# wenyuqing/panacea

Measured on AMD Instinct MI355X. Metric: denoising steps/s (6-view x 8-frame 256x512), higher is better.
Workload: dtype f16; 1 GPU; BASELINE config 3: Panacea+ stage-2 UNet+ControlNet, CFG 2 x 8 frames, 6 views, latent 32x384, hint 256x3072, Euler/LegacyDDPM 50-step schedule; precision=precise: split(stream,gn_stt,ff_out,stem,gn_head,gnt)+e4m3-lo, parallelism=single, graph=False, streams=2, hoisted_step_invariants=False, fused_step_tail=True

## Files before the change

### panacea_amd/build.py

```python
from __future__ import annotations

import hashlib
import os
import shutil
import subprocess
import sys
from pathlib import Path

PKG = Path(__file__).resolve().parent
ROOT = PKG.parent
CSRC = PKG / "csrc"
LIBDIR = PKG / "lib"
LIB = LIBDIR / "libpanacea_hip.so"
SOURCES = ["gemm.hip", "gemm_plain.hip", "gemm_conv3x3.hip", "gemm_stencil_tile.hip", "gemm_conv1d.hip", "attn.hip", "attn_split.hip", "norm.hip", "misc.hip"]
HEADERS = [CSRC / "common.h", CSRC / "gemm_kernel.h", ROOT / "include" / "panacea_hip.h"]
FLAGS = ["--offload-arch=gfx950", "-O3", "-std=c++17", "-fPIC", "-Wall", "-Wno-unused-function",
         "-I", str(ROOT / "include"), "-I", str(CSRC)]


def _hipcc() -> str:
    for cand in (os.environ.get("HIPCC"), shutil.which("hipcc"), "/opt/rocm/bin/hipcc"):
        if cand and Path(cand).exists():
            return cand
    raise RuntimeError("hipcc not found (expected /opt/rocm/bin/hipcc)")


def _digest() -> str:
    h = hashlib.sha256()
    for f in [CSRC / s for s in SOURCES] + HEADERS:
        h.update(f.read_bytes())
    h.update(" ".join(f.replace(str(ROOT), "<root>") for f in FLAGS).encode())
    return h.hexdigest()


def library_digest(lib: Path = LIB):
    try:
        blob = Path(lib).read_bytes()
    except OSError:
        return None
    i = blob.find(_DIGEST_MARK)
    if i < 0:
        return None
    j = blob.find(b"\0", i)
    return blob[i + len(_DIGEST_MARK):j].decode(errors="replace")


_DIGEST_MARK = b"pnc-build-digest:"
# ... 40 lines not shown
```

### panacea_amd/csrc/gemm.hip

```cpp
#include "gemm_kernel.h"
#include <math.h>
#include <mutex>

namespace pnc_gemm {

int dispatch_plain(const PncGemmParams& p, unsigned epi, hipStream_t st, bool* ln_fused);
int dispatch_conv3x3(const PncGemmParams& p, unsigned epi, hipStream_t st);
int dispatch_conv1d(const PncGemmParams& p, unsigned epi, hipStream_t st);

__device__ __attribute__((aligned(16))) float g_phi_table[2 * PHI_N];

const float* phi_table_device(hipStream_t st, int* rc) {
    static std::mutex mu;
    static const float* dev_ptr[64] = {};
    int dev = 0;
    (void)hipGetDevice(&dev);
    std::lock_guard<std::mutex> lock(mu);
    const float*& ptr = dev_ptr[dev & 63];
    *rc = PNC_OK;
    if (ptr) return ptr;
    hipStreamCaptureStatus cs = hipStreamCaptureStatusNone;
    if (hipStreamIsCapturing(st, &cs) == hipSuccess && cs != hipStreamCaptureStatusNone) { *rc = PNC_EINVAL; return nullptr; }
    static float host[2 * PHI_N];
    auto phi = [](double x) { return 0.5 * (1.0 + erf(x * 0.70710678118654752440)); };
    for (int i = 0; i < PHI_N; ++i) {
        const double x0 = (double)PHI_X0 + (double)i / PHI_SCALE, x1 = (double)PHI_X0 + (double)(i + 1) / PHI_SCALE;
        host[2 * i] = (float)phi(x0);
        host[2 * i + 1] = (float)(phi(x1) - phi(x0));
    }
    void* d = nullptr;
    if (hipMemcpyToSymbol(HIP_SYMBOL(g_phi_table), host, sizeof(host)) != hipSuccess ||
        hipGetSymbolAddress(&d, HIP_SYMBOL(g_phi_table)) != hipSuccess) {
        *rc = (int)hipGetLastError();
        return nullptr;
    }
    ptr = reinterpret_cast<const float*>(d);
    return ptr;
}

__global__ __launch_bounds__(256) void splitk_reduce_kernel(const PncGemmParams p, const int ksplit) {
    const int n8 = p.N >> 3;
// ... 126 lines not shown
    if (p.a_mode != PNC_A_CONV3X3 && p.x_halo_off) return PNC_EINVAL;
    if (p.gn_part && (p.a_mode != PNC_A_CONV1D_T || !p.out32 || (p.N % 64) || (p.ldc32 % 4) || p.out16t || p.geglu)) return PNC_EINVAL;
    if (p.act != PNC_ACT_NONE && p.act != PNC_ACT_SILU && p.act != PNC_ACT_GELU) return PNC_EINVAL;
    if (p.ldw != 0 && (p.ldw < p.K || p.ldw % 8)) return PNC_EALIGN;
    if (p.rowbias && (p.rb_rows <= 0 || p.rb_mod <= 0)) return PNC_EINVAL;
    if (p.geglu) {
        if ((p.N % 64) || p.out16t || p.out32 || p.res1 || p.res2 || p.rowbias || p.act != PNC_ACT_NONE || !p.out16)
            return PNC_EINVAL;
        if ((p.ldc16 % 8) || !al16(p.out16) || (p.out16_lo && !al16(p.out16_lo)) || (p.bias && !al16(p.bias)))
            return PNC_EALIGN;
    }
    if (p.out16t && ((p.n_split % 128) || p.t_rows <= 0 || p.N <= 32)) return PNC_EINVAL;
    if (p.out16_lo && !p.out16) return PNC_EINVAL;
    if ((p.a_lo_fmt != PNC_LO_F16 && p.a_lo_fmt != PNC_LO_E4M3) || (p.out_lo_fmt != PNC_LO_F16 && p.out_lo_fmt != PNC_LO_E4M3))
        return PNC_EINVAL;
    if (p.out16_lo && p.out_lo_fmt == PNC_LO_E4M3 && p.geglu) return PNC_EINVAL;
    if (p.A_lo && p.a_lo_fmt == PNC_LO_E4M3) {
        if (!p.W_lo || p.w_lo_exp < 1 || p.w_lo_exp > 254) return PNC_EINVAL;
        if ((uintptr_t)p.W_lo & 15) return PNC_EALIGN;
        if (p.K % 16 || (p.ldw_lo != 0 && (p.ldw_lo < p.K || p.ldw_lo % 16))) return PNC_EALIGN;
        if (p.a_mode == PNC_A_PLAIN ? (p.lda % 16 != 0) : (p.Cin % 64 != 0)) return PNC_EALIGN;
    }
    if (!p.out32 && !p.out16 && !p.out16t) return PNC_EINVAL;
    if (p.ln_out16) {
        if (!p.out32 || p.geglu || p.out16t || !p.ln_gamma || !p.ln_beta) return PNC_EINVAL;
        if (p.N % 4 || p.N > 4 * 64 * 12 || p.ldc32 % 4 || p.ldln % 4 || p.ldln < p.N) return PNC_EINVAL;
        if (!al16(p.out32) || !al16(p.ln_gamma) || !al16(p.ln_beta) || (((uintptr_t)p.ln_out16) & 7)) return PNC_EALIGN;
    }
    return PNC_OK;
}

extern "C" int pnc_abi_version(void) { return PNC_ABI_VERSION; }

extern "C" int64_t pnc_gemm_workspace_floats(const PncGemmParams* pp) {
    if (!pp || pp->struct_bytes != (int32_t)sizeof(PncGemmParams)) return 0;
    if (pp->M <= 0 || pp->N <= 0 || pp->K <= 0) return 0;
    if (pp->N <= 32 && !pp->geglu) return 0;
    const int ks = splitk_slices(*pp);
    return ks > 1 ? (int64_t)ks * pp->M * pp->N : 0;
}

static unsigned epilogue_with_ln(const PncGemmParams& p) {
    unsigned epi = select_epilogue(p);
    if (p.ln_out16 && p.a_mode == PNC_A_PLAIN && (epi == E_O32 || epi == (E_RB | E_O32) || epi == (E_R1 | E_O32)) &&
        (p.ldln % 8 == 0) && al16(p.ln_out16) && (pnc_get_option(PNC_OPT_GEMM_FUSE_LN) & 1))
        epi |= E_LN;
    return epi;
}

static void normalise(PncGemmParams& p) {
    if (!p.out16t) p.n_split = p.N;
    if (p.ldw == 0) p.ldw = p.K;
    if (p.ldw_lo == 0) p.ldw_lo = p.K;
    if (!p.res1 && p.res2) { p.res1 = p.res2; p.ldr1 = p.ldr2; p.res2 = nullptr; }
}

extern "C" int pnc_gemm_fuses_layernorm(const PncGemmParams* pp) {
    if (!pp || validate(*pp) != PNC_OK || !pp->ln_out16) return 0;
    PncGemmParams p = *pp;
    normalise(p);
    if (!(epilogue_with_ln(p) & E_LN)) return 0;
    const TileChoice tc = choose_tile(p);
    return ln_whole_rows(p, tc) ? 1 : 0;
}

extern "C" int pnc_gemm_f16(const PncGemmParams* pp, void* stream) {
    if (!pp) return PNC_EINVAL;
    const int rc = validate(*pp);
    if (rc != PNC_OK) return rc;
    PncGemmParams p = *pp;
    normalise(p);
    const unsigned epi = epilogue_with_ln(p);
// ... 15 lines not shown
```

### panacea_amd/csrc/gemm_conv1d.hip

```cpp
#include "gemm_kernel.h"

namespace pnc_gemm {

static bool gn_stats_in_epilogue(const PncGemmParams& p, const TileChoice& tc) {
    const int cpg = p.N / 32;
    return tc.tile == T_256x320 && (p.N % 320) == 0 && (160 % cpg) == 0 && (cpg % 2) == 0 && (p.Npix % 64) == 0 && (p.M % 64) == 0 &&
           pnc_get_option(PNC_OPT_GEMM_GN_STATS) != 0;
}

int dispatch_conv1d(const PncGemmParams& p, unsigned epi, hipStream_t st) {
    constexpr int AM = PNC_A_CONV1D_T;
    TileChoice tc = choose_tile(p);
    if (tc.tile == T_128x32) epi = E_GENERIC;
    if (p.gn_part) {
        int rc = PNC_EINVAL;
        bool fused = gn_stats_in_epilogue(p, tc);
        if (fused) {
            switch (epi) {
                case E_R1 | E_RB | E_O32: rc = launch<AM, 256, 320, 4, 2, 2, false, E_R1 | E_RB | E_O32 | E_GS>(p, st); break;
                case E_R1 | E_R2 | E_O32: rc = launch<AM, 256, 320, 4, 2, 2, false, E_R1 | E_R2 | E_O32 | E_GS>(p, st); break;
                case E_R1 | E_R2 | E_O32 | E_O16: rc = launch<AM, 256, 320, 4, 2, 2, false, E_R1 | E_R2 | E_O32 | E_O16 | E_GS>(p, st); break;
                default: fused = false;
            }
        }
        if (fused) return rc;
        PncGemmParams q = p;
        q.gn_part = nullptr;
        rc = dispatch_conv1d(q, epi, st);
        if (rc != PNC_OK) return rc;
        return pnc_groupnorm_stats(p.out32, p.ldc32, p.M / p.Npix, p.Npix, p.N, 64, p.gn_part, st);
    }
    switch (epi) {
        case E_R1 | E_RB | E_O32: return launch_tile<AM, E_R1 | E_RB | E_O32>(p, st, tc);
        case E_R1 | E_R2 | E_O32: return launch_tile<AM, E_R1 | E_R2 | E_O32>(p, st, tc);
        case E_R1 | E_R2 | E_O32 | E_O16: return launch_tile<AM, E_R1 | E_R2 | E_O32 | E_O16>(p, st, tc);
        default: return launch_tile<AM, E_GENERIC>(p, st, tc);
    }
}

}

PNC_DEFINE_TU_COLLECT(gemm_conv1d)
```

### panacea_amd/csrc/gemm_kernel.h

```cpp
#pragma once
#include "common.h"
#include <atomic>
#include <utility>

namespace pnc_gemm {

constexpr int BK = 64;
constexpr int BK8 = 128;
typedef int i32x4 __attribute__((ext_vector_type(4)));
typedef int i32x8 __attribute__((ext_vector_type(8)));
constexpr int E8M0_LO_INV = 127 - 11;

enum : unsigned {
    E_R1 = 1,
    E_R2 = 2,
    E_RB = 4,
    E_O32 = 8,
    E_O16 = 16,
    E_VT = 32,
    E_GEGLU = 64,
    E_GENERIC = 128,
    E_GELU = 256,
    E_LN = 512,
    E_GS = 1024
// ... 114 lines not shown
    for (int e = 0; e < 8; ++e) o[e] = (half_t)v[e];
    *reinterpret_cast<half8v*>(out16 + off) = o;
    if (out16_lo) {
        float r[8];
#pragma unroll
        for (int e = 0; e < 8; ++e) r[e] = (v[e] - (float)o[e]) * LO_SCALE;
        if (lo_fmt == PNC_LO_E4M3) {
            uint2 w;
            w.x = pack4_e4m3(r[0], r[1], r[2], r[3]);
            w.y = pack4_e4m3(r[4], r[5], r[6], r[7]);
            *reinterpret_cast<uint2*>(reinterpret_cast<char*>(out16_lo) + off) = w;
        } else {
            half8v l;
#pragma unroll
            for (int e = 0; e < 8; ++e) l[e] = (half_t)r[e];
            *reinterpret_cast<half8v*>(reinterpret_cast<half_t*>(out16_lo) + off) = l;
        }
    }
}

struct RowLinear {
    int mw;
    __device__ __forceinline__ int operator()(int lr) const { return mw + lr; }
};
template <int TWS>
struct RowHalo {
    int base, W, lr0;
    __device__ __forceinline__ int operator()(int lr) const {
        const int R = lr0 + lr;
        return base + (R >> TWS) * W + (R & ((1 << TWS) - 1));
    }
};

template <int MI, int NI, unsigned EPI, class RM = RowLinear>
__device__ __forceinline__ void epi_fast(const PncGemmParams& p, f32x16 (&acc)[MI][NI], float* ep, int lane,
                                         RM rmap, int nw, int ncols, float2* ln_mine = nullptr,
                                         const float2* ln_partner = nullptr, float* gs_tab = nullptr) {
    constexpr bool R1 = (EPI & E_R1) != 0, R2 = (EPI & E_R2) != 0, RB = (EPI & E_RB) != 0;
    constexpr bool O32 = (EPI & E_O32) != 0, O16 = (EPI & E_O16) != 0, LN = (EPI & E_LN) != 0;
    constexpr bool GS = (EPI & E_GS) != 0;
    static_assert(!GS || (O32 && !LN), "statistics of the fp32 output; not next to the fused LayerNorm");
    const int cpg = GS ? (p.N >> 5) : 1;
    if constexpr (GS) {
        gs_tab[lane] = 0.0f;
        if (lane + 64 < NI * 16) gs_tab[lane + 64] = 0.0f;
    }
    static_assert(!LN || O32, "the fused LayerNorm normalises the fp32 output it has just written");
    constexpr bool HAS_X = R1 || RB, HAS_Y = R1 && (R2 || RB);
    static_assert(!(R2 && !R1), "a single residual is passed as res1");
    static_assert(!(R1 && R2 && RB), "three added streams run the generic epilogue");
    constexpr int ENI = NI < 2 ? NI : 2;
    constexpr int EPITCH = ENI * 32 + 4;
    constexpr int NJ = (NI + ENI - 1) / ENI, NS = NJ * MI;
    constexpr int NPMAX = ENI == 2 ? 4 : 2;
    half_t* out16 = reinterpret_cast<half_t*>(p.out16);
    void* out16_lo = p.out16_lo;
    constexpr bool GELU = (EPI & E_GELU) != 0;
    const bool silu = (!HAS_X) && (p.act == PNC_ACT_SILU);
    const f32x4 z4 = {0.0f, 0.0f, 0.0f, 0.0f};
    f32x4 x0[NPMAX], x1[NPMAX], y0[NPMAX], y1[NPMAX];
    if constexpr (LN) {
        if (lane < MI * 32) ln_mine[lane] = make_float2(0.0f, 0.0f);
    }

    auto load_xy = [&](auto s_, auto ps_) {
        constexpr int s = decltype(s_)::value, ps = decltype(ps_)::value;
        constexpr int jc = (s / MI) * ENI, i = s % MI, cw = (NI - jc) < ENI ? (NI - jc) : ENI;
        constexpr int CPL = cw * 4, RPP = 64 / CPL;
        const int cl = lane % CPL, rl = lane / CPL;
        const int ncol = nw + jc * 32 + cl * 8;
        const int m = rmap(i * 32 + ps * RPP + rl);
        const bool on = (m < p.M) && (ncol < ncols);
        if constexpr (HAS_X) {
            x0[ps] = z4; x1[ps] = z4;
            if (on) {
                const float* xp = R1 ? p.res1 + (int64_t)m * p.ldr1 + ncol
                                     : p.rowbias + (int64_t)((m / p.rb_rows) % p.rb_mod) * p.N + ncol;
                x0[ps] = ld4(xp); x1[ps] = ld4(xp + 4);
// ... 85 lines not shown
            if constexpr (GS) {
                if (on) {
#pragma unroll
                    for (int k = 0; k < 4; ++k) {
                        gP[k] += v[2 * k] + v[2 * k + 1];
                        gQ[k] += fmaf(v[2 * k], v[2 * k], v[2 * k + 1] * v[2 * k + 1]);
                    }
                }
            }
            if (!on) return;
            if constexpr (O32) {
                float* op = p.out32 + (int64_t)m * p.ldc32 + ncol;
                const f32x4 o0 = {v[0], v[1], v[2], v[3]}, o1 = {v[4], v[5], v[6], v[7]};
                *reinterpret_cast<f32x4*>(op) = o0;
                *reinterpret_cast<f32x4*>(op + 4) = o1;
            }
            if constexpr (O16) store_h8(out16, out16_lo, (int64_t)m * p.ldc16 + ncol, v, p.out_lo_fmt);
        });
        if constexpr (GS) {
            const int nA = min(8, (ncol / cpg + 1) * cpg - ncol);
            float sA = 0.0f, qA = 0.0f, sB = 0.0f, qB = 0.0f;
#pragma unroll
            for (int k = 0; k < 4; ++k) {
                const bool a = 2 * k < nA;
                sA += a ? gP[k] : 0.0f; qA += a ? gQ[k] : 0.0f;
                sB += a ? 0.0f : gP[k]; qB += a ? 0.0f : gQ[k];
            }
#pragma unroll
            for (int o = CPL; o < 64; o <<= 1) {
                sA += __shfl_xor(sA, o, 64); qA += __shfl_xor(qA, o, 64);
                sB += __shfl_xor(sB, o, 64); qB += __shfl_xor(qB, o, 64);
            }
            if (lane < CPL) {
                f32x4* e = reinterpret_cast<f32x4*>(gs_tab + (jc * 4 + cl) * 4);
                f32x4 t = *e;
                t[0] += sA; t[1] += qA; t[2] += sB; t[3] += qB;
                *e = t;
            }
        }
        if constexpr (LN) {
            asm volatile("s_waitcnt lgkmcnt(0)" ::: "memory");
            static_for<cw>([&](auto j_) {
                constexpr int j = decltype(j_)::value;
#pragma unroll
                for (int r = 0; r < 16; ++r)
                    acc[i][jc + j][r] = ep[mfma32_row(r, lane) * EPITCH + j * 32 + (lane & 31)];
            });
        }
    });
    if constexpr (GS) {
        asm volatile("s_waitcnt lgkmcnt(0)" ::: "memory");
        const int m_first = rmap(0);
        if (lane < (NI * 32) / cpg && m_first < p.M) {
            const int c0 = (lane * cpg) >> 3, c1 = ((lane + 1) * cpg - 1) >> 3;
            float S = 0.0f, Q = 0.0f;
            for (int c = c0; c <= c1; ++c) {
                const f32x4 t = *reinterpret_cast<const f32x4*>(gs_tab + c * 4);
                const bool first = (c * 8) / cpg == lane;
                S += first ? t[0] : t[2];
                Q += first ? t[1] : t[3];
            }
            const float n = (float)(MI * 32 * cpg);
            const float mean = S / n;
            const int f = m_first / p.Npix, chunk = (m_first - f * p.Npix) / (MI * 32), nrec = p.Npix / (MI * 32);
            float* o = p.gn_part + ((int64_t)(f * nrec + chunk) * 32 + nw / cpg + lane) * 3;
            o[0] = n; o[1] = mean; o[2] = fmaxf(Q - S * mean, 0.0f);
        }
    }
    if constexpr (LN) {
        __syncthreads();
        half_t* lnout = reinterpret_cast<half_t*>(p.ln_out16);
        const float invn = 1.0f / (float)p.N;
        static_for<NS>([&](auto s_) {
            constexpr int s = decltype(s_)::value, jc = (s / MI) * ENI, i = s % MI;
            constexpr int cw = (NI - jc) < ENI ? (NI - jc) : ENI;
            constexpr int CPL = cw * 4, RPP = 64 / CPL, NP = 32 / RPP;
            const int cl = lane % CPL, rl = lane / CPL;
            const int ncol = nw + jc * 32 + cl * 8;
            const bool col_on = ncol < ncols;
            f32x4 g0 = z4, g1 = z4, h0 = z4, h1 = z4;
            if (col_on) {
                g0 = ld4(p.ln_gamma + ncol); g1 = ld4(p.ln_gamma + ncol + 4);
                h0 = ld4(p.ln_beta + ncol); h1 = ld4(p.ln_beta + ncol + 4);
// ... 1522 lines not shown
```

### panacea_amd/csrc/misc.hip

```cpp
#include "common.h"
#include <atomic>

namespace {

constexpr int SM_MAXM = 16;

__global__ __launch_bounds__(256) void linear_smallm_kernel(const float* __restrict__ a, int lda,
                                                            const half_t* __restrict__ W,
                                                            const float* __restrict__ bias,
                                                            float* __restrict__ out, int ldo, int M, int N,
                                                            int K, int silu_in, int silu_out) {
    const int lane = threadIdx.x & 63;
    const int n = blockIdx.x * 4 + (threadIdx.x >> 6);
    if (n >= N) return;
    float acc[SM_MAXM];
#pragma unroll
    for (int m = 0; m < SM_MAXM; ++m) acc[m] = 0.0f;
    for (int k0 = lane * 8; k0 < K; k0 += 64 * 8) {
        const half8v w = *reinterpret_cast<const half8v*>(W + (int64_t)n * K + k0);
        float wf[8];
#pragma unroll
        for (int e = 0; e < 8; ++e) wf[e] = (float)w[e];
#pragma unroll
        for (int m = 0; m < SM_MAXM; ++m) {
// ... 496 lines not shown
    const float inv = 1.0f / (((red[4] + red[5]) + red[6]) + red[7]);
#pragma unroll
    for (int j = 0; j < 16; ++j) {
        const int c = tid + j * 256;
        if (c < nv) {
            half4v h;
#pragma unroll
            for (int e = 0; e < 4; ++e) h[e] = (half_t)(v[j][e] * inv);
            *reinterpret_cast<half4v*>(prow + c * 4) = h;
        }
    }
}

extern "C" int pnc_softmax_rows_f16(const float* s, int64_t lds, int M, int N, float scale, int causal, int n_valid,
                                    void* p16, int64_t ldp, void* stream) {
    if (!s || !p16 || M < 1 || N < 4 || N > 16384 || (N & 3) || n_valid > N) return PNC_EINVAL;
    if (n_valid <= 0) n_valid = N;
    if ((lds & 3) || (ldp & 3) || lds < N || ldp < N) return PNC_EINVAL;
    if (((uintptr_t)s & 15) || ((uintptr_t)p16 & 7)) return PNC_EALIGN;
    hipLaunchKernelGGL(softmax_rows_kernel, dim3((unsigned)M), dim3(256), 0, reinterpret_cast<hipStream_t>(stream), s, lds, N,
                       scale, causal, n_valid, reinterpret_cast<half_t*>(p16), ldp);
    return pnc_launch_status();
}

extern "C" int pnc_cast_f16(const float* x, int64_t n, void* y16, void* y16_lo, int lo_fmt, void* stream) {
    return pnc_add_f32(x, nullptr, n, nullptr, y16, y16_lo, lo_fmt, stream);
}

PNC_DEFINE_TU_COLLECT(misc)
void pnc_tu_collect_gemm(unsigned int*, hipStream_t);
void pnc_tu_collect_gemm_plain(unsigned int*, hipStream_t);
void pnc_tu_collect_gemm_conv3x3(unsigned int*, hipStream_t);
void pnc_tu_collect_gemm_conv1d(unsigned int*, hipStream_t);
void pnc_tu_collect_gemm_stencil_tile(unsigned int*, hipStream_t);
void pnc_tu_collect_norm(unsigned int*, hipStream_t);

extern "C" int pnc_range_monitor_collect(unsigned int* out, void* stream) {
    if (!out) return PNC_EINVAL;
    hipStream_t st = reinterpret_cast<hipStream_t>(stream);
    pnc_tu_collect_gemm(out, st);
    pnc_tu_collect_gemm_plain(out, st);
    pnc_tu_collect_gemm_conv3x3(out, st);
    pnc_tu_collect_gemm_conv1d(out, st);
    pnc_tu_collect_gemm_stencil_tile(out, st);
    pnc_tu_collect_norm(out, st);
    pnc_tu_collect_misc(out, st);
    return pnc_launch_status();
}
```

### panacea_amd/hip.py

```python
from __future__ import annotations

import ctypes as C
import re
from pathlib import Path
from typing import Optional

import torch

PKG = Path(__file__).resolve().parent
LIB_PATH = PKG / "lib" / "libpanacea_hip.so"
HEADER = PKG.parent / "include" / "panacea_hip.h"

A_PLAIN, A_CONV3X3, A_CONV1D_T = 0, 1, 2
ACT_NONE, ACT_SILU, ACT_GELU = 0, 1, 2
ABI_VERSION = 8
LO_F16, LO_E4M3 = 0, 1
LO_DTYPE = {LO_F16: torch.float16, LO_E4M3: torch.uint8}


def lo_fmt(t: Optional[torch.Tensor]) -> int:
    if t is None or t.dtype == torch.float16:
        return LO_F16
    if t.dtype == torch.uint8:
        return LO_E4M3
# ... 132 lines not shown
        lib = C.CDLL(str(LIB_PATH))
    except OSError as e:
        raise HipLibraryError(f"cannot load {LIB_PATH}: {e}") from e
    if not os.environ.get("PANACEA_HIP_LIB"):
        from . import build as _build
        try:
            lib.pnc_build_digest.restype = C.c_char_p
            have = lib.pnc_build_digest().decode()
        except AttributeError:
            have = "(a library older than pnc_build_digest)"
        if _build.CSRC.exists() and have != _build._digest():
            raise HipLibraryError(f"{LIB_PATH} was built from other sources ({have[:12]}) than panacea_amd/csrc holds now "
                                  f"({_build._digest()[:12]}); rebuild it with `python -m panacea_amd.build`")
    for name, (res, args) in _SIGNATURES.items():
        try:
            fn = getattr(lib, name)
        except AttributeError as e:
            raise HipLibraryError(f"{LIB_PATH} does not export {name}; rebuild the extension") from e
        fn.restype = res
        fn.argtypes = args
    if lib.pnc_abi_version() != ABI_VERSION:
        raise HipLibraryError(f"{LIB_PATH} implements C-ABI version {lib.pnc_abi_version()}, this binding needs "
                              f"{ABI_VERSION}; rebuild the extension (`python -m panacea_amd.build --force`)")
    _lib = lib
    return lib


OPT_GEMM_TAIL_SPLIT, OPT_GEMM_TILE, OPT_ATTN_VARIANT, OPT_ATTN_DMA, OPT_GEMM_FUSE_LN, OPT_GEMM_GROUP_M, OPT_STENCIL_TILES = 0, 1, 2, 3, 4, 5, 6
OPT_GEMM_PERSIST = 7
OPT_ATTN_DEFER_MAX = 8
OPT_GEMM_GN_STATS = 9
OPT_GEMM_STAGGER = 10
OPT_ATTN_SUM_TRIGGER = 11


def build_digest() -> str:
    return load().pnc_build_digest().decode()


def set_option(option: int, value: int) -> int:
    if not 0 <= option <= OPT_ATTN_SUM_TRIGGER:
        raise PncError(f"unknown library option {option}")
    return load().pnc_set_option(option, value)


CU_MASK_PATTERNS = {
    "even-odd": ([0x55555555] * 8, [0xAAAAAAAA] * 8),
    "nibbles": ([0x0F0F0F0F] * 8, [0xF0F0F0F0] * 8),
    "halves": ([0xFFFFFFFF] * 4 + [0] * 4, [0] * 4 + [0xFFFFFFFF] * 4),
}


def masked_stream(words) -> "torch.cuda.Stream":
    rt = None
    for line in open("/proc/self/maps"):
        if "libamdhip64" in line:
            rt = C.CDLL(line.split()[-1])
            break
    if rt is None:
        raise PncError("the HIP runtime is not loaded")
    rt.hipExtStreamCreateWithCUMask.argtypes = [C.POINTER(C.c_void_p), C.c_uint32, C.POINTER(C.c_uint32)]
    rt.hipExtStreamCreateWithCUMask.restype = C.c_int
    st = C.c_void_p()
    arr = (C.c_uint32 * len(words))(*words)
    rc = rt.hipExtStreamCreateWithCUMask(C.byref(st), C.c_uint32(len(words)), arr)
    if rc != 0:
# ... 46 lines not shown

def _stream() -> int:
    return torch.cuda.current_stream().cuda_stream


def _ptr(t: Optional[torch.Tensor], dtype=None, name: str = "operand") -> Optional[int]:
    if t is None:
        return None
    if not t.is_cuda:
        raise PncError("panacea_amd kernels need tensors resident in HBM (got a CPU tensor); "
                       "there is no CPU fallback")
    if t.device.index != torch.cuda.current_device():
        raise PncError(f"{name} lives on cuda:{t.device.index} but the current device is cuda:{torch.cuda.current_device()}: "
                       "select the tensors' device (torch.cuda.device / set_device) before calling the kernels")
    if dtype is not None and t.dtype != dtype:
        raise PncError(f"{name}: expected {dtype}, got {t.dtype}")
    return t.data_ptr()


def gemm(a16: torch.Tensor, w16: torch.Tensor, *, M: int, N: int, K: int, lda: int = 0,
         a_mode: int = A_PLAIN, conv: Optional[dict] = None, tconv: Optional[dict] = None,
         bias: Optional[torch.Tensor] = None, rowbias: Optional[torch.Tensor] = None,
         rb_rows: int = 0, rb_mod: int = 0,
         res1: Optional[torch.Tensor] = None, ldr1: int = 0,
         res2: Optional[torch.Tensor] = None, ldr2: int = 0,
         out32: Optional[torch.Tensor] = None, ldc32: int = 0,
         out16: Optional[torch.Tensor] = None, ldc16: int = 0,
         out16t: Optional[torch.Tensor] = None, ldt: int = 0, t_rows: int = 0, t_gstride: int = 0,
         n_split: int = 0, act: int = ACT_NONE, geglu: bool = False,
         a16_lo: Optional[torch.Tensor] = None, out16_lo: Optional[torch.Tensor] = None, w_ld: int = 0,
         w_lo: Optional[tuple] = None,
         ln_gamma: Optional[torch.Tensor] = None, ln_beta: Optional[torch.Tensor] = None,
         ln_out16: Optional[torch.Tensor] = None, ldln: int = 0, ln_eps: float = 1e-5, ln_in_library: bool = False,
         gn_part: Optional[torch.Tensor] = None):
    p = GemmParams()
    p.struct_bytes = C.sizeof(GemmParams)
    f16, f32 = torch.float16, torch.float32
    p.A, p.W = _ptr(a16, f16, "a16"), _ptr(w16, f16, "w16")
    p.a_lo_fmt, p.out_lo_fmt = lo_fmt(a16_lo), lo_fmt(out16_lo)
    p.A_lo, p.out16_lo = _ptr(a16_lo, LO_DTYPE[p.a_lo_fmt], "a16_lo"), _ptr(out16_lo, LO_DTYPE[p.out_lo_fmt], "out16_lo")
    if p.a_lo_fmt == LO_E4M3:
        if w_lo is None:
            raise PncError("an e4m3 lo plane needs the e4m3 copy of the weights (w_lo = engine.pk_lo8(w16))")
        p.W_lo, p.w_lo_exp = _ptr(w_lo[0], torch.uint8, "w_lo"), int(w_lo[1])
        p.ldw_lo = w_lo[0].shape[-1]
    p.M, p.N, p.K, p.lda, p.a_mode, p.ldw = M, N, K, lda, a_mode, w_ld
    if ln_out16 is not None:
        p.ln_gamma, p.ln_beta, p.ln_out16 = _ptr(ln_gamma, torch.float32, "ln_gamma"), _ptr(ln_beta, torch.float32, "ln_beta"), \
            _ptr(ln_out16, torch.float16, "ln_out16")
        p.ldln, p.ln_eps = ldln, ln_eps
    if conv:
        p.Cin, p.Hin, p.Win = conv["Cin"], conv["Hin"], conv["Win"]
        p.Hout, p.Wout = conv["Hout"], conv["Wout"]
        p.stride, p.upsample = conv.get("stride", 1), int(conv.get("upsample", 0))
        p.conv_pad_br = int(conv.get("pad_br", 0))
        p.x_halo_off = int(conv.get("x_halo_off", 0))
    if tconv:
        p.Cin, p.T, p.Npix = tconv["C"], tconv["T"], tconv["Npix"]
        p.t_halo = int(tconv.get("halo", 0))
    p.gn_part = _ptr(gn_part, f32, "gn_part")
    p.bias, p.rowbias, p.rb_rows, p.rb_mod = _ptr(bias, f32, "bias"), _ptr(rowbias, f32, "rowbias"), rb_rows, rb_mod
    p.res1, p.ldr1, p.res2, p.ldr2 = _ptr(res1, f32, "res1"), ldr1, _ptr(res2, f32, "res2"), ldr2
    p.out32, p.ldc32, p.out16, p.ldc16 = _ptr(out32, f32, "out32"), ldc32, _ptr(out16, f16, "out16"), ldc16
    p.out16t, p.ldt, p.t_rows, p.t_gstride = _ptr(out16t, f16, "out16t"), ldt, t_rows, t_gstride
    p.n_split = n_split if out16t is not None else N
    p.act, p.geglu = act, int(geglu)
    lib = load()
    nws = lib.pnc_gemm_workspace_floats(C.byref(p))
    ws = None
    if nws > 0:
        ws = torch.empty(nws, device=a16.device, dtype=torch.float32)
        p.ws, p.ws_floats = _ptr(ws), nws
    fam = ("gemm_plain", "gemm_conv3x3", "gemm_conv1d_t")[a_mode]
    trailing_ln = ln_out16 is not None and not ln_in_library and not lib.pnc_gemm_fuses_layernorm(C.byref(p))
    if trailing_ln:
        p.ln_gamma = p.ln_beta = p.ln_out16 = None
    _check(_timed(fam, 2.0 * M * N * K, 0.0, lib.pnc_gemm_f16, C.byref(p), _stream()), "pnc_gemm_f16")
    if trailing_ln:
        layernorm(out32, ldc32, M, N, ln_gamma, ln_beta, ln_eps, ln_out16, ldln)


def _attn_params(p, q, ldq, k, ldk, vt, ldvt, vt_gstride, o, ldo, groups, heads, H, W, views, kvH, kvW, kv_views,
                 kv_rows_per_group, q_per_kv, kv_valid, segs, scale, causal):
    p.q, p.ldq, p.k, p.ldk = _ptr(q), ldq, _ptr(k), ldk
    p.vt, p.ldvt, p.vt_gstride, p.o, p.ldo = _ptr(vt), ldvt, vt_gstride, _ptr(o), ldo
    p.groups, p.heads, p.H, p.W, p.views = groups, heads, H, W, views
    p.kvH, p.kvW, p.kv_views = kvH, kvW, kv_views
    p.kv_rows_per_group, p.q_per_kv, p.kv_valid = kv_rows_per_group, q_per_kv, kv_valid
    for v, s in enumerate(segs):
        p.nseg[v] = len(s)
        for j, u in enumerate(s):
            p.seg[v][j] = u
    p.scale, p.causal = scale, int(causal)


def attn_views(q, ldq, k, ldk, vt, ldvt, vt_gstride, o, ldo, *, groups, heads, H, W, views,
               kvH, kvW, kv_views, kv_rows_per_group, q_per_kv, kv_valid, segs, scale, causal=False, k_halo=None, vt_halo=None):
    p = AttnParams()
    if k_halo is not None:
        for i in range(2):
            p.k_halo[i], p.vt_halo[i] = _ptr(k_halo[i]), _ptr(vt_halo[i])
# ... 163 lines not shown
```

Baseline: 6.633 steps/s.

## Add frame-blocked temporal conv1d GEMM kernel sharing A tiles across three taps

Adds a specialised kernel for the temporal 3-tap conv1d GEMM. Each 256-row tile holds all T frames of a pixel block, so one A stage in LDS is reused for all three taps instead of being reloaded per tap. GroupNorm statistics are written as per-32-row half records into a workspace and reduced by a small finish kernel. This costs an extra launch and a workspace allocation, and falls back to the old path when shapes do not fit.

```diff
diff --git a/panacea_amd/build.py b/panacea_amd/build.py
--- a/panacea_amd/build.py
+++ b/panacea_amd/build.py
@@ -12,7 +12,7 @@
 CSRC = PKG / "csrc"
 LIBDIR = PKG / "lib"
 LIB = LIBDIR / "libpanacea_hip.so"
-SOURCES = ["gemm.hip", "gemm_plain.hip", "gemm_conv3x3.hip", "gemm_stencil_tile.hip", "gemm_conv1d.hip", "attn.hip", "attn_split.hip", "norm.hip", "misc.hip"]
+SOURCES = ["gemm.hip", "gemm_plain.hip", "gemm_conv3x3.hip", "gemm_stencil_tile.hip", "gemm_conv1d.hip", "gemm_conv1d_frames.hip", "attn.hip", "attn_split.hip", "norm.hip", "misc.hip"]
 HEADERS = [CSRC / "common.h", CSRC / "gemm_kernel.h", ROOT / "include" / "panacea_hip.h"]
 FLAGS = ["--offload-arch=gfx950", "-O3", "-std=c++17", "-fPIC", "-Wall", "-Wno-unused-function",
          "-I", str(ROOT / "include"), "-I", str(CSRC)]
diff --git a/panacea_amd/csrc/gemm.hip b/panacea_amd/csrc/gemm.hip
--- a/panacea_amd/csrc/gemm.hip
+++ b/panacea_amd/csrc/gemm.hip
@@ -7,6 +7,7 @@
 int dispatch_plain(const PncGemmParams& p, unsigned epi, hipStream_t st, bool* ln_fused);
 int dispatch_conv3x3(const PncGemmParams& p, unsigned epi, hipStream_t st);
 int dispatch_conv1d(const PncGemmParams& p, unsigned epi, hipStream_t st);
+int64_t conv1d_frames_ws_floats(const PncGemmParams& p, unsigned epi);
 
 __device__ __attribute__((aligned(16))) float g_phi_table[2 * PHI_N];
 
@@ -199,12 +200,20 @@
 
 extern "C" int pnc_abi_version(void) { return PNC_ABI_VERSION; }
 
+static void normalise(PncGemmParams& p);
+
 extern "C" int64_t pnc_gemm_workspace_floats(const PncGemmParams* pp) {
     if (!pp || pp->struct_bytes != (int32_t)sizeof(PncGemmParams)) return 0;
     if (pp->M <= 0 || pp->N <= 0 || pp->K <= 0) return 0;
     if (pp->N <= 32 && !pp->geglu) return 0;
     const int ks = splitk_slices(*pp);
-    return ks > 1 ? (int64_t)ks * pp->M * pp->N : 0;
+    if (ks > 1) return (int64_t)ks * pp->M * pp->N;
+    if (pp->a_mode == PNC_A_CONV1D_T && pp->gn_part && validate(*pp) == PNC_OK) {
+        PncGemmParams p = *pp;
+        normalise(p);
+        return conv1d_frames_ws_floats(p, select_epilogue(p));
+    }
+    return 0;
 }
 
 static unsigned epilogue_with_ln(const PncGemmParams& p) {
diff --git a/panacea_amd/csrc/gemm_conv1d.hip b/panacea_amd/csrc/gemm_conv1d.hip
--- a/panacea_amd/csrc/gemm_conv1d.hip
+++ b/panacea_amd/csrc/gemm_conv1d.hip
@@ -1,6 +1,9 @@
 #include "gemm_kernel.h"
 
 namespace pnc_gemm {
+
+int conv1d_frames_tile(const PncGemmParams& p, unsigned epi, const TileChoice& tc);
+int dispatch_conv1d_frames(const PncGemmParams& p, unsigned epi, int tile, hipStream_t st);
 
 static bool gn_stats_in_epilogue(const PncGemmParams& p, const TileChoice& tc) {
     const int cpg = p.N / 32;
@@ -12,6 +15,7 @@
     constexpr int AM = PNC_A_CONV1D_T;
     TileChoice tc = choose_tile(p);
     if (tc.tile == T_128x32) epi = E_GENERIC;
+    if (const int ft = conv1d_frames_tile(p, epi, tc)) return dispatch_conv1d_frames(p, epi, ft, st);
     if (p.gn_part) {
         int rc = PNC_EINVAL;
         bool fused = gn_stats_in_epilogue(p, tc);
diff --git a/panacea_amd/csrc/gemm_conv1d_frames.hip b/panacea_amd/csrc/gemm_conv1d_frames.hip
--- /dev/null
+++ b/panacea_amd/csrc/gemm_conv1d_frames.hip
@@ -0,0 +1,325 @@
+#include "gemm_kernel.h"
+
+namespace pnc_gemm {
+
+struct RowFrames {
+    int base, Npix, lt, lr0;
+    __device__ __forceinline__ int operator()(int lr) const {
+        const int R = lr0 + lr, blk = R >> 5;
+        return base + (blk & ((1 << lt) - 1)) * Npix + ((blk >> lt) << 5) + (R & 31);
+    }
+};
+
+template <int BN, unsigned EPI>
+__global__ __launch_bounds__(512) void conv1d_frames_kernel(const PncGemmParams pin, const int lt, const int nfull, const int tail_f) {
+    PncGemmParams p = pin;
+    constexpr int BM = 256, WGM = 4, WGN = 2, NW = 8, MI = 2, NI = BN / WGN / 32, RPI = NW * 8, A_IT = BM / RPI, B_IT = BN / RPI;
+    constexpr int A_BYTES = BM * 128, B_BYTES = BN * 128, W_BASE = 2 * A_BYTES;
+    constexpr int EPITCH = 2 * 32 + 4;
+    static_assert(BN % RPI == 0 && NI >= 2, "column tile of whole DMA row groups");
+    static_assert(NW * (32 * EPITCH * 4) + NW * MI * NI * 64 <= 2 * (A_BYTES + B_BYTES), "epilogue staging + statistics tables fit the ring");
+    extern __shared__ __attribute__((aligned(16))) char smem[];
+    const half_t* __restrict__ A = reinterpret_cast<const half_t*>(p.A);
+    const half_t* __restrict__ A_lo = reinterpret_cast<const half_t*>(p.A_lo);
+    const half_t* __restrict__ Wt = reinterpret_cast<const half_t*>(p.W);
+    const int T = 1 << lt, ppt = BM >> lt;
+    const int tiles_n = p.N / BN, pb_n = p.Npix / ppt;
+    int tile, part = 0;
+    if ((int)blockIdx.x < nfull) tile = xcd_remap(blockIdx.x, nfull);
+    else {
+        const int j = (int)blockIdx.x - nfull;
+        tile = nfull + j / tail_f; part = j - (j / tail_f) * tail_f;
+    }
+    const bool split_rows = ((int)blockIdx.x >= nfull) && (tail_f > 1);
+    const int tn = tile % tiles_n, tm = tile / tiles_n;
+    const int smp = tm / pb_n, pb = tm - smp * pb_n;
+    const int base_m = smp * T * p.Npix + pb * ppt, n0 = tn * BN;
+    const int nsl = p.Cin >> 6;
+    const bool lo8 = A_lo && p.a_lo_fmt == PNC_LO_E4M3;
+    const int ntiles = 3 * nsl;
+    const int nt_lo = A_lo ? (lo8 ? (p.K + BK8 - 1) / BK8 : ntiles) : 0;
+    const int ngl = (nt_lo + 2) / 3;
+    const int ntot = ntiles + nt_lo;
+
+    const int tid = threadIdx.x, lane = tid & 63;
+    const int wave = __builtin_amdgcn_readfirstlane(tid >> 6);
+    const int wm = wave / WGN, wn = wave % WGN;
+    const int srow = wave * 8 + (lane >> 3);
+    const int schunk = (lane & 7) ^ ((srow >> 1) & 7);
+    const int rows_lo = split_rows ? part * (BM / tail_f) : 0;
+    const int rows_hi = split_rows ? rows_lo + BM / tail_f : BM;
+    const bool wave_on = (wm * (MI * 32) >= rows_lo) && (wm * (MI * 32) < rows_hi);
+    unsigned aoff[A_IT], woff[B_IT];
+#pragma unroll
+    for (int i = 0; i < A_IT; ++i) {
+        const int r = i * RPI + srow, blk = r >> 5;
+        const int rel = ((blk & (T - 1)) * p.Npix + ((blk >> lt) << 5) + (r & 31)) * p.Cin;
+        aoff[i] = (r >= rows_lo - 32 && r < rows_hi + 32) ? (unsigned)(rel + schunk * 8) * 2u : PNC_BUF_OOB;
+    }
+#pragma unroll
+    for (int i = 0; i < B_IT; ++i) {
+        const int nl = i * RPI + srow;
+        woff[i] = (n0 + nl < p.N) ? (unsigned)(nl * p.ldw + schunk * 8) * 2u : PNC_BUF_OOB;
+    }
+    const int64_t a_origin = (int64_t)base_m * p.Cin;
+    const buffer_rsrc_t rs_a = make_rsrc(A + a_origin, 0x7FFFFF00u);
+    const buffer_rsrc_t rs_alo = make_rsrc(lo8 ? static_cast<const void*>(reinterpret_cast<const char*>(p.A_lo) + a_origin)
+                                               : static_cast<const void*>((A_lo ? A_lo : A) + a_origin), 0x7FFFFF00u);
+    const buffer_rsrc_t rs_w = make_rsrc(Wt + (int64_t)n0 * p.ldw, 0x7FFFFF00u);
+    const buffer_rsrc_t rs_wlo = make_rsrc(lo8 ? static_cast<const void*>(reinterpret_cast<const char*>(p.W_lo) + (int64_t)n0 * p.ldw_lo)
+                                               : static_cast<const void*>(Wt + (int64_t)n0 * p.ldw), 0x7FFFFF00u);
+
+    auto a_stage_of = [&](int j) { return (j < nt_lo ? j / 3 : ngl + (j - nt_lo) / 3) & 1; };
+    auto issue = [&](int j) __attribute__((always_inline)) {
+        const bool lo = j < nt_lo;
+        const int jj = lo ? j : j - nt_lo;
+        const int grp = jj / 3;
+        const bool with_a = jj - grp * 3 == 0;
+        char* sa = smem + a_stage_of(j) * A_BYTES + wave * 1024;
+        char* sb = smem + W_BASE + (j & 1) * B_BYTES + wave * 1024;
+        if (lo && lo8) {
+            int schunk8 = schunk, srow8 = srow;
+            asm volatile("" : "+v"(schunk8), "+v"(srow8));
+            const unsigned ks8 = (unsigned)jj * BK8;
+            const bool k_on = jj * BK8 + schunk8 * 16 < p.K;
+#pragma unroll
+            for (int i = 0; i < B_IT; ++i)
+                glds16_buf(rs_wlo, (k_on && woff[i] != PNC_BUF_OOB) ? (unsigned)((i * RPI + srow8) * p.ldw_lo + schunk8 * 16) : PNC_BUF_OOB,
+                           ks8, sb + i * (RPI * 128));
+            if (with_a) {
+                const bool c_on = grp * BK8 + schunk8 * 16 < p.Cin;
+#pragma unroll
+                for (int i = 0; i < A_IT; ++i)
+                    glds16_buf(rs_alo, (c_on && aoff[i] != PNC_BUF_OOB) ? (aoff[i] >> 1) + (unsigned)schunk8 * 8u : PNC_BUF_OOB,
+                               (unsigned)grp * BK8, sa + i * (RPI * 128));
+            }
+            return;
+        }
+        const unsigned ks = (unsigned)jj * (BK * 2);
+#pragma unroll
+        for (int i = 0; i < B_IT; ++i) glds16_buf(rs_w, woff[i], ks, sb + i * (RPI * 128));
+        if (with_a) {
+            const buffer_rsrc_t rs = lo ? rs_alo : rs_a;
+#pragma unroll
+            for (int i = 0; i < A_IT; ++i) glds16_buf(rs, aoff[i], (unsigned)grp * (BK * 2), sa + i * (RPI * 128));
+        }
+    };
+
+    f32x16 acc[MI][NI];
+#pragma unroll
+    for (int i = 0; i < MI; ++i)
+#pragma unroll
+        for (int j = 0; j < NI; ++j)
+#pragma unroll
+            for (int r = 0; r < 16; ++r) acc[i][j][r] = 0.0f;
+
+    const int frow = lane & 31, fk = lane >> 5;
+    auto a_block = [&](int tap, int (&sblk)[MI], bool (&on)[MI]) {
+#pragma unroll
+        for (int i = 0; i < MI; ++i) {
+            const int b = wm * MI + i, tt = (b & (T - 1)) + tap - 1;
+            on[i] = tt >= 0 && tt < T;
+            sblk[i] = on[i] ? b + tap - 1 : b;
+        }
+    };
+    auto compute = [&](int j, int mid_issue) {
+        const int jj = j < nt_lo ? j : j - nt_lo;
+        const int tap = jj - (jj / 3) * 3;
+        const char* sa = smem + a_stage_of(j) * A_BYTES;
+        const char* sb = smem + W_BASE + (j & 1) * B_BYTES;
+        int sblk[MI];
+        bool on[MI];
+        a_block(tap, sblk, on);
+#pragma unroll
+        for (int ks = 0; ks < BK / 16; ++ks) {
+            half8v af[MI], bf[NI];
+#pragma unroll
+            for (int i = 0; i < MI; ++i)
+                af[i] = *reinterpret_cast<const half8v*>(sa + lds_off128(sblk[i] * 32 + frow, ks * 2 + fk));
+#pragma unroll
+            for (int jn = 0; jn < NI; ++jn)
+                bf[jn] = *reinterpret_cast<const half8v*>(sb + lds_off128(wn * (NI * 32) + jn * 32 + frow, ks * 2 + fk));
+#pragma unroll
+            for (int i = 0; i < MI; ++i) {
+                if (on[i]) {
+#pragma unroll
+                    for (int jn = 0; jn < NI; ++jn)
+                        acc[i][jn] = __builtin_amdgcn_mfma_f32_32x32x16_f16(af[i], bf[jn], acc[i][jn], 0, 0, 0);
+                }
+            }
+            if (ks == 1 && mid_issue >= 0) issue(mid_issue);
+        }
+    };
+    auto compute8 = [&](int j) {
+        const char* sa = smem + a_stage_of(j) * A_BYTES;
+        const char* sb = smem + W_BASE + (j & 1) * B_BYTES;
+#pragma unroll
+        for (int w = 0; w < 2; ++w) {
+            const int u = 2 * j + w;
+            if (u < ntiles) {
+                const int s = u / 3, tap = u - s * 3, cb = (s & 1) * 4 + fk * 2;
+                int sblk[MI];
+                bool on[MI];
+                a_block(tap, sblk, on);
+                i32x8 af[MI];
+#pragma unroll
+                for (int i = 0; i < MI; ++i) {
+                    const int row = sblk[i] * 32 + frow;
+                    const i32x4 a0 = *reinterpret_cast<const i32x4*>(sa + lds_off128(row, cb));
+                    const i32x4 a1 = *reinterpret_cast<const i32x4*>(sa + lds_off128(row, cb + 1));
+                    af[i] = __builtin_shufflevector(a0, a1, 0, 1, 2, 3, 4, 5, 6, 7);
+                }
+#pragma unroll
+                for (int jn = 0; jn < NI; ++jn) {
+                    const int row = wn * (NI * 32) + jn * 32 + frow;
+                    const i32x4 b0 = *reinterpret_cast<const i32x4*>(sb + lds_off128(row, w * 4 + fk * 2));
+                    const i32x4 b1 = *reinterpret_cast<const i32x4*>(sb + lds_off128(row, w * 4 + fk * 2 + 1));
+                    const i32x8 bf = __builtin_shufflevector(b0, b1, 0, 1, 2, 3, 4, 5, 6, 7);
+#pragma unroll
+                    for (int i = 0; i < MI; ++i) {
+                        if (on[i])
+                            acc[i][jn] = __builtin_amdgcn_mfma_scale_f32_32x32x64_f8f6f4(af[i], bf, acc[i][jn], 0, 0, 0, E8M0_LO_INV, 0, p.w_lo_exp);
+                    }
+                    __builtin_amdgcn_sched_barrier(0);
+                }
+            }
+        }
+    };
+
+    issue(0);
+    __syncthreads();
+    const bool late = wave >= 4 && wave_on && ntot >= 8;
+    const int n8 = lo8 ? nt_lo : 0;
+    for (int j = 0; j < n8; ++j) {
+        if (j + 1 < ntot) issue(j + 1);
+        if (wave_on) compute8(j);
+        __syncthreads();
+    }
+    for (int j = n8; j < ntot; ++j) {
+        const bool nxt = j + 1 < ntot;
+        if (nxt && !late) issue(j + 1);
+        if (wave_on) {
+            compute(j, (nxt && late) ? j + 1 : -1);
+            if (!lo8 && j + 1 == nt_lo) {
+#pragma unroll
+                for (int i = 0; i < MI; ++i)
+#pragma unroll
+                    for (int jn = 0; jn < NI; ++jn)
+#pragma unroll
+                        for (int r = 0; r < 16; ++r) acc[i][jn][r] *= LO_INV;
+            }
+        }
+        __syncthreads();
+    }
+
+    if (!wave_on) return;
+    const int nw = n0 + wn * (NI * 32);
+    float* ep = reinterpret_cast<float*>(smem) + wave * (32 * EPITCH);
+    float* gs_tab = reinterpret_cast<float*>(smem) + NW * (32 * EPITCH) + wave * (MI * NI * 16);
+    __syncthreads();
+    epi_fast<MI, NI, EPI, RowFrames, true>(p, acc, ep, lane, RowFrames{base_m, p.Npix, lt, wm * (MI * 32)}, nw, p.N, nullptr, nullptr,
+                                           (EPI & E_GS) ? gs_tab : nullptr);
+}
+
+__global__ __launch_bounds__(256) void gn_half_finish_kernel(const float* __restrict__ ws, int N, int nrec, float* __restrict__ part) {
+    const int idx = blockIdx.x * 256 + threadIdx.x;
+    if (idx >= nrec * 32) return;
+    const int rec = idx >> 5, g = idx & 31, cpg = N >> 5, nch = N >> 3;
+    const f32x4* h0 = reinterpret_cast<const f32x4*>(ws) + (int64_t)(2 * rec) * nch;
+    const f32x4* h1 = h0 + nch;
+    const int c0 = (g * cpg) >> 3, c1 = ((g + 1) * cpg - 1) >> 3;
+    float S = 0.0f, Q = 0.0f;
+    for (int c = c0; c <= c1; ++c) {
+        const f32x4 t = h0[c] + h1[c];
+        const bool first = (c * 8) / cpg == g;
+        S += first ? t[0] : t[2];
+        Q += first ? t[1] : t[3];
+    }
+    const float n = (float)(64 * cpg);
+    const float mean = S / n;
+    float* o = part + (int64_t)idx * 3;
+    o[0] = n; o[1] = mean; o[2] = fmaxf(Q - S * mean, 0.0f);
+}
+
+template <int BN, unsigned EPI>
+static int launch_frames(const PncGemmParams& p, hipStream_t st) {
+    constexpr int lds = 2 * (256 + BN) * 128;
+    static std::atomic<unsigned char> attr_done[64];
+    int dev = 0;
+    (void)hipGetDevice(&dev);
+    auto kern = conv1d_frames_kernel<BN, EPI>;
+    if (!attr_done[dev & 63].load(std::memory_order_acquire)) {
+        (void)hipFuncSetAttribute(reinterpret_cast<const void*>(kern), hipFuncAttributeMaxDynamicSharedMemorySize, lds);
+        attr_done[dev & 63].store(1, std::memory_order_release);
+    }
+    const int tiles = (p.M / 256) * (p.N / BN);
+    int nfull = tiles, tail_f = 1;
+    tail_split<256, 4, lds>(tiles, nfull, tail_f);
+    hipLaunchKernelGGL(kern, dim3(nfull + (tiles - nfull) * tail_f), dim3(512), lds, st, p, p.T == 8 ? 3 : 2, nfull, tail_f);
+    return pnc_launch_status();
+}
+
+static bool frames_gn_fused(const PncGemmParams& p, int tile) {
+    const int cpg = p.N / 32;
+    return tile == T_256x320 && (160 % cpg) == 0 && (cpg % 2) == 0 && (p.Npix % 64) == 0 && pnc_get_option(PNC_OPT_GEMM_GN_STATS) != 0;
+}
+
+int conv1d_frames_tile(const PncGemmParams& p, unsigned epi, const TileChoice& tc) {
+    if ((pnc_get_option(PNC_OPT_STENCIL_TILES) & 8) || p.a_mode != PNC_A_CONV1D_T || tc.ksplit != 1) return 0;
+    if ((tc.tile != T_256x320 || p.N % 320) && (tc.tile != T_256x256 || p.N % 256)) return 0;
+    if ((p.T != 4 && p.T != 8) || p.t_halo || (p.Cin % 64) || (p.Npix % (256 / p.T))) return 0;
+    if ((int64_t)p.T * p.Npix * p.Cin * 2 >= ((int64_t)1 << 31) - 65536) return 0;
+    if (epi != (E_R1 | E_RB | E_O32) && epi != (E_R1 | E_R2 | E_O32) && epi != (E_R1 | E_R2 | E_O32 | E_O16)) return 0;
+    if (p.gn_part && frames_gn_fused(p, tc.tile) && !(p.ws && p.ws_floats >= (int64_t)p.M * p.N / 64)) return 0;
+    return tc.tile;
+}
+
+int64_t conv1d_frames_ws_floats(const PncGemmParams& p, unsigned epi) {
+    if (!p.gn_part) return 0;
+    PncGemmParams q = p;
+    q.ws = nullptr; q.ws_floats = 0;
+    const TileChoice tc = choose_tile(q);
+    q.gn_part = nullptr;
+    return (conv1d_frames_tile(q, epi, tc) && frames_gn_fused(p, tc.tile)) ? (int64_t)p.M * p.N / 64 : 0;
+}
+
+int dispatch_conv1d_frames(const PncGemmParams& p, unsigned epi, int tile, hipStream_t st) {
+    if (p.gn_part && !frames_gn_fused(p, tile)) {
+        PncGemmParams q = p;
+        q.gn_part = nullptr;
+        const int rc = dispatch_conv1d_frames(q, epi, tile, st);
+        if (rc != PNC_OK) return rc;
+        return pnc_groupnorm_stats(p.out32, p.ldc32, p.M / p.Npix, p.Npix, p.N, 64, p.gn_part, st);
+    }
+    int rc = PNC_EINVAL;
+    if (p.gn_part) {
+        switch (epi) {
+            case E_R1 | E_RB | E_O32: rc = launch_frames<320, E_R1 | E_RB | E_O32 | E_GS>(p, st); break;
+            case E_R1 | E_R2 | E_O32: rc = launch_frames<320, E_R1 | E_R2 | E_O32 | E_GS>(p, st); break;
+            case E_R1 | E_R2 | E_O32 | E_O16: rc = launch_frames<320, E_R1 | E_R2 | E_O32 | E_O16 | E_GS>(p, st); break;
+            default: break;
+        }
+        if (rc != PNC_OK) return rc;
+        const int nrec = p.M / 64;
+        hipLaunchKernelGGL(gn_half_finish_kernel, dim3((nrec * 32 + 255) / 256), dim3(256), 0, st, p.ws, p.N, nrec, p.gn_part);
+        return pnc_launch_status();
+    }
+    if (tile == T_256x320) {
+        switch (epi) {
+            case E_R1 | E_RB | E_O32: return launch_frames<320, E_R1 | E_RB | E_O32>(p, st);
+            case E_R1 | E_R2 | E_O32: return launch_frames<320, E_R1 | E_R2 | E_O32>(p, st);
+            case E_R1 | E_R2 | E_O32 | E_O16: return launch_frames<320, E_R1 | E_R2 | E_O32 | E_O16>(p, st);
+            default: return rc;
+        }
+    }
+    switch (epi) {
+        case E_R1 | E_RB | E_O32: return launch_frames<256, E_R1 | E_RB | E_O32>(p, st);
+        case E_R1 | E_R2 | E_O32: return launch_frames<256, E_R1 | E_R2 | E_O32>(p, st);
+        case E_R1 | E_R2 | E_O32 | E_O16: return launch_frames<256, E_R1 | E_R2 | E_O32 | E_O16>(p, st);
+        default: return rc;
+    }
+}
+
+}
+
+PNC_DEFINE_TU_COLLECT(gemm_conv1d_frames)
diff --git a/panacea_amd/csrc/gemm_kernel.h b/panacea_amd/csrc/gemm_kernel.h
--- a/panacea_amd/csrc/gemm_kernel.h
+++ b/panacea_amd/csrc/gemm_kernel.h
@@ -170,7 +170,7 @@
     }
 };
 
-template <int MI, int NI, unsigned EPI, class RM = RowLinear>
+template <int MI, int NI, unsigned EPI, class RM = RowLinear, bool GSH = false>
 __device__ __forceinline__ void epi_fast(const PncGemmParams& p, f32x16 (&acc)[MI][NI], float* ep, int lane,
                                          RM rmap, int nw, int ncols, float2* ln_mine = nullptr,
                                          const float2* ln_partner = nullptr, float* gs_tab = nullptr) {
@@ -182,6 +182,11 @@
     if constexpr (GS) {
         gs_tab[lane] = 0.0f;
         if (lane + 64 < NI * 16) gs_tab[lane + 64] = 0.0f;
+        if constexpr (GSH) {
+#pragma unroll
+            for (int o = 64; o < MI * NI * 16; o += 64)
+                if (lane + o < MI * NI * 16) gs_tab[lane + o] = 0.0f;
+        }
     }
     static_assert(!LN || O32, "the fused LayerNorm normalises the fp32 output it has just written");
     constexpr bool HAS_X = R1 || RB, HAS_Y = R1 && (R2 || RB);
@@ -333,7 +338,7 @@
                 sB += __shfl_xor(sB, o, 64); qB += __shfl_xor(qB, o, 64);
             }
             if (lane < CPL) {
-                f32x4* e = reinterpret_cast<f32x4*>(gs_tab + (jc * 4 + cl) * 4);
+                f32x4* e = reinterpret_cast<f32x4*>(gs_tab + ((GSH ? i * NI * 4 : 0) + jc * 4 + cl) * 4);
                 f32x4 t = *e;
                 t[0] += sA; t[1] += qA; t[2] += sB; t[3] += qB;
                 *e = t;
@@ -349,7 +354,15 @@
             });
         }
     });
-    if constexpr (GS) {
+    if constexpr (GS && GSH) {
+        asm volatile("s_waitcnt lgkmcnt(0)" ::: "memory");
+        if (lane < NI * 4) {
+#pragma unroll
+            for (int i = 0; i < MI; ++i)
+                *reinterpret_cast<f32x4*>(p.ws + ((int64_t)(rmap(i * 32) >> 5) * (p.N >> 3) + (nw >> 3) + lane) * 4) =
+                    *reinterpret_cast<const f32x4*>(gs_tab + (i * NI * 4 + lane) * 4);
+        }
+    } else if constexpr (GS) {
         asm volatile("s_waitcnt lgkmcnt(0)" ::: "memory");
         const int m_first = rmap(0);
         if (lane < (NI * 32) / cpg && m_first < p.M) {
diff --git a/panacea_amd/csrc/misc.hip b/panacea_amd/csrc/misc.hip
--- a/panacea_amd/csrc/misc.hip
+++ b/panacea_amd/csrc/misc.hip
@@ -552,6 +552,7 @@
 void pnc_tu_collect_gemm_plain(unsigned int*, hipStream_t);
 void pnc_tu_collect_gemm_conv3x3(unsigned int*, hipStream_t);
 void pnc_tu_collect_gemm_conv1d(unsigned int*, hipStream_t);
+void pnc_tu_collect_gemm_conv1d_frames(unsigned int*, hipStream_t);
 void pnc_tu_collect_gemm_stencil_tile(unsigned int*, hipStream_t);
 void pnc_tu_collect_norm(unsigned int*, hipStream_t);
 
@@ -562,6 +563,7 @@
     pnc_tu_collect_gemm_plain(out, st);
     pnc_tu_collect_gemm_conv3x3(out, st);
     pnc_tu_collect_gemm_conv1d(out, st);
+    pnc_tu_collect_gemm_conv1d_frames(out, st);
     pnc_tu_collect_gemm_stencil_tile(out, st);
     pnc_tu_collect_norm(out, st);
     pnc_tu_collect_misc(out, st);
diff --git a/panacea_amd/hip.py b/panacea_amd/hip.py
--- a/panacea_amd/hip.py
+++ b/panacea_amd/hip.py
@@ -188,6 +188,7 @@
 OPT_GEMM_GN_STATS = 9
 OPT_GEMM_STAGGER = 10
 OPT_ATTN_SUM_TRIGGER = 11
+STENCIL_TILES_NO_CONV1D_FRAMES = 8
 
 
 def build_digest() -> str:
@@ -300,7 +301,7 @@
          w_lo: Optional[tuple] = None,
          ln_gamma: Optional[torch.Tensor] = None, ln_beta: Optional[torch.Tensor] = None,
          ln_out16: Optional[torch.Tensor] = None, ldln: int = 0, ln_eps: float = 1e-5, ln_in_library: bool = False,
-         gn_part: Optional[torch.Tensor] = None):
+         gn_part: Optional[torch.Tensor] = None, query_workspace: bool = False):
     p = GemmParams()
     p.struct_bytes = C.sizeof(GemmParams)
     f16, f32 = torch.float16, torch.float32
@@ -335,6 +336,8 @@
     p.act, p.geglu = act, int(geglu)
     lib = load()
     nws = lib.pnc_gemm_workspace_floats(C.byref(p))
+    if query_workspace:
+        return nws
     ws = None
     if nws > 0:
         ws = torch.empty(nws, device=a16.device, dtype=torch.float32)
```

After: 6.621 steps/s. No clear change (-0.2%).
